# apachepinot/pinot

Measured on NVIDIA H100. Metric: scanned rows/sec for filter+groupby(3 dims,4 aggs) @1/2/4/8 H100; %HBM BW, higher is better.
Workload: dtype f64

## Files before the change

pinot_b200/csrc/pb_device.cuh:

```cuda
#pragma once
#include <cuda_runtime.h>
#include <stdint.h>

#define PB_NTHREADS 256
#define PB_NWARPS 8
#define PB_CHUNK_DOCS 1024
#define PB_NSTAGE 2
#define PB_MAX_LEAVES 16
#define PB_MAX_NODES 32
#define PB_MAX_GROUP_BY 16
#define PB_MAX_AGGS 16
#define PB_MAX_SCAN_SLOTS 8
#define PB_MAX_AGG_FILTERS 8
#define PB_MAX_AF_LEAVES 16
#define PB_MAX_AF_NODES 48
#define PB_SPARSE_MAX 128
#define PB_OUT_CAP 256
#define PB_CAND_CAP 512
#define PB_SET_SMEM_BYTES 8192

enum { L_TRUE = 0, L_FALSE = 1, L_DICT_RANGE = 2, L_DICT_SET = 3, L_RAW_RANGE_I = 4, L_RAW_RANGE_F = 5,
       L_RAW_SET = 6, L_BITMAP = 7 };
enum { N_LEAF = 0, N_AND = 1, N_OR = 2, N_NOT = 3 };
enum { T_KEYLESS = 0, T_DENSE = 1, T_HASH = 2 };
// ... 677 lines not shown
  __device__ __forceinline__ uint32_t fcnt(int k, uint32_t slot) const { return base + 4u * ((uint32_t)(1 + k) * S + slot); }
  __device__ __forceinline__ uint32_t acc(int k, uint32_t slot) const { return base + ((((1u + n_fc) * S * 4u) + 7u) & ~7u) + 8u * ((uint32_t)k * S + slot); }
};
__host__ __device__ __forceinline__ size_t pb_smem_table_bytes(uint32_t S, int n_fc, int n_acc) {
  return ((((size_t)(1 + n_fc) * S * 4 + 7) & ~(size_t)7) + (size_t)n_acc * S * 8 + 15) & ~(size_t)15;
}

__device__ __forceinline__ void pb_accumulate_smem(const DevQuery& Q, const DevSegQuery& sq, const DevTable& t, const SmemTable& st, uint32_t doc, uint32_t fpass) {
  const int nA = Q.n_aggs;
  uint64_t slot, slot_hi;
  double vals[PB_MAX_AGGS];
  pb_gather_doc(Q, sq, doc, slot, slot_hi, vals);
  const uint32_t sl = (uint32_t)slot;
  pb_sh_add_u32(st.cnt(sl), 1u);
  for (int a = 0; a < nA; a++) {
    const int op = Q.agg_op[a];
    const int fo = Q.agg_filter_of[a];
    if (fo >= 0) {
      if (!((fpass >> fo) & 1u)) continue;
      if (st.fc_of[a] >= 0) pb_sh_add_u32(st.fcnt(st.fc_of[a], sl), 1u);
    }
    if (op == 0) continue;
    const double v = vals[a];
    if (op == 5) {
      if (t.dset[a]) { pb_dset_insert(t, a, slot, (unsigned long long)__double_as_longlong(v)); continue; }
      uint32_t id = (uint32_t)__double_as_longlong(v);
      pb_red_or_b32(&t.dc_bits[a][slot * t.dc_words[a] + (id >> 5)], 1u << (id & 31));
      continue;
    }
    const uint32_t cell = st.acc(st.acc_of[a], sl);
    if (op == 1 || op == 4) {
      unsigned long long old = pb_sh_ld_u64(cell), assumed;
      do {
        assumed = old;
        old = pb_sh_cas_u64(cell, assumed, (unsigned long long)__double_as_longlong(__longlong_as_double((long long)assumed) + v));
      } while (old != assumed);
    } else if (v == v) {
      const long long e = op == 2 ? pb_enc_f64(v) : ~pb_enc_f64(v);
      long long old = (long long)pb_sh_ld_u64(cell);
      while (e < old) {
        const long long seen = (long long)pb_sh_cas_u64(cell, (unsigned long long)old, (unsigned long long)e);
        if (seen == old) break;
        old = seen;
      }
    }
  }
}

struct DevRowKey { uint32_t off, bits; uint64_t mult; const int32_t* remap; };
struct DevRowAgg { uint32_t off, width, type, exact_int; };
struct DevRowSeg {
  const uint32_t* rows;
  uint64_t doc_base;
  int32_t table, pad;
  DevRowKey keys[PB_MAX_GROUP_BY];
  DevRowAgg aggs[PB_MAX_AGGS];
};

template <int RW>
__device__ __forceinline__ void pb_load_row(const uint32_t* __restrict__ rows, unsigned long long doc, uint32_t (&w)[RW]) {
  const uint32_t* __restrict__ row = rows + doc * (unsigned long long)RW;
  if (RW == 2) { const uint2 v = __ldg(reinterpret_cast<const uint2*>(row)); w[0] = v.x; w[1 % RW] = v.y; }
  else {
#pragma unroll
    for (int q4 = 0; q4 < RW / 4; q4++) {
      const uint4 v = __ldg(reinterpret_cast<const uint4*>(row) + q4);
      w[(4 * q4) % RW] = v.x; w[(4 * q4 + 1) % RW] = v.y; w[(4 * q4 + 2) % RW] = v.z; w[(4 * q4 + 3) % RW] = v.w;
    }
  }
#pragma unroll
  for (int k = 0; k < RW; k++) w[k] = pb_bswap32(w[k]);
}

template <int RW>
__device__ __forceinline__ uint32_t pb_row_field(const uint32_t (&w)[RW], uint32_t off, uint32_t bits) {
  const uint32_t wi = off >> 5, sh = off & 31u;
  uint32_t hi = w[0], lo = RW > 1 ? w[1 % RW] : 0u;
#pragma unroll
  for (int k = 1; k < RW; k++) if (wi == (uint32_t)k) { hi = w[k]; lo = k + 1 < RW ? w[(k + 1) % RW] : 0u; }
  return __funnelshift_l(lo, hi, sh) >> (32u - bits);
}

template <int RW>
__device__ __forceinline__ uint64_t pb_row_slot(const uint32_t (&w)[RW], const DevRowSeg& sg, int nG) {
  uint64_t slot = 0;
  for (int j = 0; j < nG; j++) {
    const DevRowKey& k = sg.keys[j];
    uint32_t id = pb_row_field<RW>(w, k.off, k.bits);
    if (k.remap) id = (uint32_t)__ldg(k.remap + id);
    slot += (uint64_t)id * k.mult;
  }
  return slot;
}

template <int RW>
__device__ __forceinline__ double pb_row_value(const uint32_t (&w)[RW], const DevRowAgg& g) {
  const uint32_t w0 = pb_row_field<RW>(w, g.off, 32u);
  if (g.width == 4) return g.type == 2 ? (double)__uint_as_float(w0) : (double)(int32_t)w0;
  const unsigned long long u = ((unsigned long long)w0 << 32) | pb_row_field<RW>(w, g.off + 32u, 32u);
  return g.type == 3 ? __longlong_as_double((long long)u) : (double)(long long)u;
}
template <int RW>
__device__ __forceinline__ long long pb_row_ivalue(const uint32_t (&w)[RW], const DevRowAgg& g) {
  const uint32_t w0 = pb_row_field<RW>(w, g.off, 32u);
  if (g.width == 4) return (long long)(int32_t)w0;
  return (long long)(((unsigned long long)w0 << 32) | pb_row_field<RW>(w, g.off + 32u, 32u));
}

template <int RW>
__device__ __forceinline__ void pb_row_aggregate_global(const DevQuery& Q, const DevRowSeg& sg, const uint32_t (&w)[RW], uint64_t slot, uint32_t doc) {
  const DevTable& t = Q.tables[sg.table];
  pb_red_add_u64(&t.rowcnt[slot], 1ull);
  if (t.first_doc) asm volatile("red.global.min.u32 [%0], %1;" ::"l"(t.first_doc + slot), "r"(doc));
  for (int a = 0; a < Q.n_aggs; a++) {
    const int op = Q.agg_op[a];
    if (op == 0) continue;
    const double v = pb_row_value<RW>(w, sg.aggs[a]);
    if (op == 1 || op == 4) pb_red_add_f64(&t.sum[a][slot], v);
    else if (v == v) pb_red_min_s64(&t.mm[a][slot], op == 2 ? pb_enc_f64(v) : ~pb_enc_f64(v));
  }
}

struct __align__(16) FilterSmemHeader {
  uint64_t full[PB_NWARPS][PB_NSTAGE];
  uint32_t slot_stride[PB_MAX_SCAN_SLOTS];
  uint32_t slot_last_rel[PB_MAX_SCAN_SLOTS];
  uint32_t n_scan_full_bytes;
  int32_t flat_and;
  int32_t n_flat;
  int32_t flat_leaf[PB_MAX_LEAVES];
  int32_t n_dense;
  int32_t pad_g;
  alignas(16) uint8_t seg[PB_SEG_FILTER_BYTES];
};

template <int U, int MIN_CTAS, int SW = 0, int SPK = 0, int RW = 0>
__global__ void __launch_bounds__(PB_NTHREADS, MIN_CTAS) pb_filter_kernel(const __grid_constant__ DevQuery Q) {
  extern __shared__ __align__(128) uint8_t smem_raw[];
  FilterSmemHeader* H = reinterpret_cast<FilterSmemHeader*>(smem_raw);
  const int tid = threadIdx.x, lane = tid & 31, warp = tid >> 5;
  uint8_t* dyn = smem_raw + ((sizeof(FilterSmemHeader) + 127) & ~(size_t)127);
  DevRowSeg* rseg = reinterpret_cast<DevRowSeg*>(dyn);
  if constexpr (RW > 0) dyn += (sizeof(DevRowSeg) + 127) & ~(size_t)127;
  uint8_t* set_cache = dyn;
  dyn += (Q.set_cache_bytes + 127) & ~127;
  uint16_t* cand = reinterpret_cast<uint16_t*>(dyn);
  dyn += Q.cand_bytes;
  const uint32_t OUT_CAP = (uint32_t)Q.out_cap, CAND_CAP = (uint32_t)Q.cand_cap;
  uint32_t* ob = reinterpret_cast<uint32_t*>(dyn) + (size_t)warp * OUT_CAP;
  dyn += (size_t)PB_NWARPS * OUT_CAP * sizeof(uint32_t);
  uint32_t out_n = 0;
  auto flush_out = [&]() {
    if (out_n == 0) return;
    __syncwarp();
    unsigned long long base = 0;
    if (lane == 0) base = atomicAdd(Q.match_count, (unsigned long long)out_n);
    base = __shfl_sync(0xffffffffu, base, 0);
    for (uint32_t i = (uint32_t)lane; i < out_n; i += 32) Q.match_list[base + i] = ob[i];
    __syncwarp();
    out_n = 0;
  };
  uint8_t* my_stages = dyn + (size_t)warp * PB_NSTAGE * Q.stage_bytes;
  const bool staged = Q.stage_bytes > 0;
  constexpr uint32_t UNIT_DOCS = U * PB_CHUNK_DOCS;

  if (lane == 0)
    for (int s = 0; s < PB_NSTAGE; s++) pb_mbar_init(&H->full[warp][s], 1);
  asm volatile("fence.mbarrier_init.release.cluster;" ::: "memory");
  __syncthreads();

  const uint64_t per = (Q.n_units + gridDim.x - 1) / gridDim.x;
  const uint64_t cta_lo = Q.unit_lo + (uint64_t)blockIdx.x * per;
  const uint64_t cta_hi = cta_lo + per < Q.unit_lo + Q.n_units ? cta_lo + per : Q.unit_lo + Q.n_units;
  if (cta_lo >= cta_hi) return;
  int seg_first = 0;
  while (seg_first + 1 < Q.n_segs && cta_lo >= Q.segs[seg_first + 1].unit_begin) seg_first++;

  uint32_t consumed = 0;
  const DevSegQuery& sq = *reinterpret_cast<const DevSegQuery*>(H->seg);
  const uint64_t l2_stream = pb_policy_evict_first();

  auto eval_leaf = [&](const DevLeaf& lf, const uint8_t* stage, uint64_t unit_doc0, int nu, const uint32_t* restrict_to, bool sparse, uint32_t* m) {
    switch (lf.kind) {
      case L_TRUE: for (int u = 0; u < nu; u++) m[u] = 0xffffffffu; return;
      case L_FALSE: for (int u = 0; u < nu; u++) m[u] = 0u; return;
      case L_DICT_RANGE: {
        const uint32_t* p = reinterpret_cast<const uint32_t*>(stage + Q.slot_off[lf.slot]);
        PredRange pr; pr.lo = lf.lo; pr.span = lf.span;
        if (sparse) { for (int u = 0; u < nu; u++) m[u] = pb_eval_dict_sparse<PredRange>(p + u * 32 * lf.bits, lf.bits, pr, lane, restrict_to[u]); return; }
        pb_eval_dict<PredRange>(p, lf.bits, pr, lane, Q.generic, nu, m);
        return;
      }
      case L_DICT_SET: {
        const uint32_t* p = reinterpret_cast<const uint32_t*>(stage + Q.slot_off[lf.slot]);
        if (lf.set_smem_off >= 0) {
          PredLut8 pl; pl.lut = set_cache + lf.set_smem_off;
          if (sparse) { for (int u = 0; u < nu; u++) m[u] = pb_eval_dict_sparse<PredLut8>(p + u * 32 * lf.bits, lf.bits, pl, lane, restrict_to[u]); return; }
          pb_eval_dict<PredLut8>(p, lf.bits, pl, lane, Q.generic, nu, m);
          return;
        }
        PredBits pb; pb.bits = lf.set_bits; pb.excl = (uint32_t)lf.exclusive;
        if (sparse) { for (int u = 0; u < nu; u++) m[u] = pb_eval_dict_sparse<PredBits>(p + u * 32 * lf.bits, lf.bits, pb, lane, restrict_to[u]); return; }
        pb_eval_dict<PredBits>(p, lf.bits, pb, lane, Q.generic, nu, m);
        return;
      }
      case L_RAW_RANGE_I:
      case L_RAW_RANGE_F:
      case L_RAW_SET: {
        const uint32_t* p = reinterpret_cast<const uint32_t*>(stage + Q.slot_off[lf.slot]);
        for (int u = 0; u < nu; u++) m[u] = pb_eval_raw(p + u * (PB_CHUNK_DOCS / 4) * lf.raw_width, lf, lane);
        return;
      }
      default: {
        for (int u = 0; u < nu; u++) {
          uint32_t w = __ldg(lf.bitmap + (unit_doc0 >> 5) + u * 32 + lane);
          m[u] = lf.exclusive ? ~w : w;
        }
        return;
      }
    }
  };

  for (int sgi = seg_first; sgi < Q.n_segs; sgi++) {
    if (Q.segs[sgi].unit_begin >= cta_hi) break;
    __syncthreads();
    {
      const uint32_t* src = reinterpret_cast<const uint32_t*>(&Q.segs[sgi]);
      uint32_t* dst = reinterpret_cast<uint32_t*>(H->seg);
      for (int i = tid; i < (int)(PB_SEG_FILTER_BYTES / 4); i += PB_NTHREADS) dst[i] = src[i];
      if constexpr (RW > 0) {
        const uint32_t* rsrc = reinterpret_cast<const uint32_t*>(Q.row_segs + sgi);
        uint32_t* rdst = reinterpret_cast<uint32_t*>(rseg);
        for (int i = tid; i < (int)(sizeof(DevRowSeg) / 4); i += PB_NTHREADS) rdst[i] = rsrc[i];
      }
      __syncthreads();
      if (tid < sq.n_scan) {
        const uint32_t stride = (uint32_t)(UNIT_DOCS / 8) * (uint32_t)sq.scan[tid].bits_per_doc;
        H->slot_stride[tid] = stride;
        const uint64_t total = sq.scan[tid].bytes_total;
        H->slot_last_rel[tid] = total >= (uint64_t)stride + 16 ? (uint32_t)((total - stride - 16) / stride) + 1 : 0u;
      }
      if (tid == 96) {
        uint32_t t = 0;
        for (int c = 0; c < sq.n_scan; c++) t += (uint32_t)(UNIT_DOCS / 8) * (uint32_t)sq.scan[c].bits_per_doc + 16;
        H->n_scan_full_bytes = t;
      }
      if (tid == 64) {
        int nl = 0; bool flat = true;
        for (int n = 0; n < sq.n_nodes; n++) {
          if (sq.node_kind[n] == N_LEAF) { if (nl < PB_MAX_LEAVES) H->flat_leaf[nl] = sq.node_arg[n]; nl++; }
          else if (!(sq.node_kind[n] == N_AND && n == sq.n_nodes - 1 && sq.node_arg[n] == nl)) flat = false;
        }
        int nd = 0;
        if (flat && nl <= PB_MAX_LEAVES) {
          auto key = [&](int l) { return sq.leaves[l].est_permille + (sq.leaves[l].gather ? 4096 : 0); };
          for (int a = 1; a < nl; a++) {
            int x = H->flat_leaf[a]; int b = a - 1;
            while (b >= 0 && key(H->flat_leaf[b]) > key(x)) { H->flat_leaf[b + 1] = H->flat_leaf[b]; b--; }
            H->flat_leaf[b + 1] = x;
          }
          for (int a = 0; a < nl; a++) if (!sq.leaves[H->flat_leaf[a]].gather) nd++;
        }
        H->flat_and = flat ? 1 : 0;
        H->n_flat = nl;
        H->n_dense = nd;
      }
      for (int l = 0; l < PB_MAX_LEAVES; l++) {
        const DevLeaf& lf = sq.leaves[l];
        if (lf.kind == L_DICT_SET && lf.set_smem_off >= 0) {
          for (int i = tid; i < lf.set_card; i += PB_NTHREADS)
            set_cache[lf.set_smem_off + i] = (uint8_t)(((__ldg(lf.set_bits + (i >> 5)) >> (i & 31)) & 1u) ^ (uint32_t)lf.exclusive);
        }
      }
      __syncthreads();
    }
    const uint64_t seg_lo = sq.unit_begin > cta_lo ? sq.unit_begin : cta_lo;
    const uint64_t seg_end = sq.unit_begin + sq.n_units;
    const uint64_t seg_hi = seg_end < cta_hi ? seg_end : cta_hi;
    const uint64_t first = seg_lo + warp;
    const uint32_t n_mine = first < seg_hi ? (uint32_t)((seg_hi - first + PB_NWARPS - 1) / PB_NWARPS) : 0u;
    const uint32_t rel0 = (uint32_t)(first - sq.unit_begin);
    const int n_scan = sq.n_scan;
    unsigned long long matched = 0;
    uint32_t min_last_rel = 0xffffffffu;
    for (int c = 0; c < n_scan; c++) min_last_rel = min(min_last_rel, H->slot_last_rel[c]);

    auto issue = [&](uint32_t k, uint32_t seq) {
      const uint32_t rel = rel0 + k * PB_NWARPS;
      const int st = (int)(seq % PB_NSTAGE);
      uint8_t* dst = my_stages + (size_t)st * Q.stage_bytes;
      uint64_t* bar = &H->full[warp][st];
      if (__builtin_expect(rel < min_last_rel, 1)) {
        pb_mbar_expect_tx(bar, H->n_scan_full_bytes);
        for (int c = 0; c < n_scan; c++) {
          const uint32_t stride = H->slot_stride[c];
          pb_tma_load_1d_hint(dst + Q.slot_off[c], sq.scan[c].base + (uint64_t)rel * stride, stride + 16, bar, l2_stream);
        }
        return;
      }
      uint32_t total = 0;
      uint32_t nbytes[PB_MAX_SCAN_SLOTS];
      for (int c = 0; c < n_scan; c++) {
        const uint64_t off = (uint64_t)rel * H->slot_stride[c];
        const uint64_t want = (uint64_t)H->slot_stride[c] + 16;
        const uint64_t avail = sq.scan[c].bytes_total - off;
        nbytes[c] = (uint32_t)((want < avail ? want : avail) & ~(uint64_t)15);
        total += nbytes[c];
      }
      pb_mbar_expect_tx(bar, total);
      for (int c = 0; c < n_scan; c++)
        pb_tma_load_1d(dst + Q.slot_off[c], sq.scan[c].base + (uint64_t)rel * H->slot_stride[c], nbytes[c], bar);
    };

    if (staged && Q.use_tma && lane == 0)
      for (uint32_t k = 0; k < PB_NSTAGE - 1 && k < n_mine; k++) issue(k, consumed + k);

    for (uint32_t k = 0; k < n_mine; k++) {
      const uint64_t unit_doc0 = (uint64_t)(rel0 + k * PB_NWARPS) * UNIT_DOCS;
      const int st = (int)(consumed % PB_NSTAGE);
      uint8_t* stage = my_stages + (size_t)st * Q.stage_bytes;
      if (staged) {
        if (__builtin_expect(Q.use_tma != 0, 1)) {
          if (lane == 0 && k + PB_NSTAGE - 1 < n_mine) issue(k + PB_NSTAGE - 1, consumed + PB_NSTAGE - 1);
          pb_mbar_wait(&H->full[warp][st], (consumed / PB_NSTAGE) & 1u);
        } else {
          for (int c = 0; c < n_scan; c++) {
            const uint64_t off = (uint64_t)(rel0 + k * PB_NWARPS) * H->slot_stride[c];
            const uint64_t want = (uint64_t)H->slot_stride[c] + 16;
            const uint64_t avail = sq.scan[c].bytes_total - off;
            const uint64_t n = (want < avail ? want : avail) & ~(uint64_t)15;
            const uint4* s4 = reinterpret_cast<const uint4*>(sq.scan[c].base + off);
            uint4* d4 = reinterpret_cast<uint4*>(stage + Q.slot_off[c]);
            for (uint32_t i = lane; i < (uint32_t)(n / 16); i += 32) d4[i] = __ldg(s4 + i);
          }
          __syncwarp();
        }
      }
      consumed++;

      uint32_t mask[U], tmp[U];
      int nu = 0;
      const uint32_t nd_rel = (uint32_t)sq.num_docs - (uint32_t)unit_doc0;
      nu = nd_rel >= (uint32_t)U * PB_CHUNK_DOCS ? U : (int)((nd_rel + PB_CHUNK_DOCS - 1) / PB_CHUNK_DOCS);
#pragma unroll
      for (int u = 0; u < U; u++) {
        const uint32_t d = (uint32_t)u * PB_CHUNK_DOCS + 32u * (uint32_t)lane;
        mask[u] = nd_rel >= d + 32u ? 0xffffffffu : (nd_rel <= d ? 0u : ((1u << (nd_rel - d)) - 1u));
      }
      const int n_cand_leaves = H->flat_and ? H->n_flat - H->n_dense : 0;
      if constexpr (SW > 0) {
        const DevLeaf& lf = sq.leaves[H->flat_leaf[0]];
        const uint32_t* p = reinterpret_cast<const uint32_t*>(stage + Q.slot_off[lf.slot]);
        if constexpr (SPK == 0) {
          PredRange pr; pr.lo = lf.lo; pr.span = lf.span;
#pragma unroll
          for (int u = 0; u < U; u++) if (u < nu) mask[u] &= pb_eval_dict_w<SW, PredRange>(p + u * 32 * SW, pr, lane);
        } else {
          PredLut8 pl; pl.lut = set_cache + lf.set_smem_off;
#pragma unroll
          for (int u = 0; u < U; u++) if (u < nu) mask[u] &= pb_eval_dict_w<SW, PredLut8>(p + u * 32 * SW, pl, lane);
        }
      } else if (__builtin_expect(H->flat_and != 0, 1)) {
        const int nl = H->n_dense;
        for (int i = 0; i < nl; i++) {
          uint32_t pc = 0;
#pragma unroll
          for (int u = 0; u < U; u++) pc += (uint32_t)__popc(mask[u]);
          const bool sparse = i > 0 && !Q.generic && __reduce_add_sync(0xffffffffu, pc) <= (uint32_t)Q.sparse_max * U;
          eval_leaf(sq.leaves[H->flat_leaf[i]], stage, unit_doc0, nu, mask, sparse, tmp);
          uint32_t any = 0;
#pragma unroll
          for (int u = 0; u < U; u++) { if (u < nu) mask[u] &= tmp[u]; any |= mask[u]; }
          if (sparse && !__any_sync(0xffffffffu, any != 0)) break;
        }
      } else {
        uint32_t stack[PB_MAX_LEAVES][U];
        const uint32_t all[2] = {0xffffffffu, 0xffffffffu};
        int sp = 0;
        for (int n = 0; n < sq.n_nodes; n++) {
          const int kind = sq.node_kind[n], arg = sq.node_arg[n];
          if (kind == N_LEAF) { eval_leaf(sq.leaves[arg], stage, unit_doc0, nu, all, false, stack[sp]); sp++; }
          else if (kind == N_NOT) { for (int u = 0; u < nu; u++) stack[sp - 1][u] = ~stack[sp - 1][u]; }
          else {
            for (int u = 0; u < nu; u++) {
              uint32_t r = stack[sp - arg][u];
              for (int i = 1; i < arg; i++) r = (kind == N_AND) ? (r & stack[sp - arg + i][u]) : (r | stack[sp - arg + i][u]);
              stack[sp - arg][u] = r;
            }
            sp -= arg - 1;
          }
        }
        if (sp > 0) for (int u = 0; u < nu; u++) mask[u] &= stack[0][u];
      }
      __syncwarp();

      uint32_t cnt = 0;
#pragma unroll
      for (int u = 0; u < U; u++) cnt += (uint32_t)__popc(mask[u]);
      const uint32_t mx = __reduce_max_sync(0xffffffffu, cnt);
      if (mx == 0) continue;
      uint32_t excl = 0, total = 0;
      const uint32_t lt = (1u << lane) - 1u;
      if (mx <= 4) {
        for (uint32_t kk = 1; kk <= mx; kk++) {
          const uint32_t b = __ballot_sync(0xffffffffu, cnt >= kk);
          excl += __popc(b & lt);
          total += __popc(b);
        }
      } else {
        uint32_t incl = cnt;
#pragma unroll
        for (int o = 1; o < 32; o <<= 1) { uint32_t t = __shfl_up_sync(0xffffffffu, incl, o); if (lane >= o) incl += t; }
        total = __shfl_sync(0xffffffffu, incl, 31);
        excl = incl - cnt;
      }
      const uint32_t gunit0 = (uint32_t)(sq.doc_base + unit_doc0);
      if (RW == 0 && n_cand_leaves == 0) {
        if (__builtin_expect(total > OUT_CAP, 0)) {
          unsigned long long base = 0;
          if (lane == 0) base = atomicAdd(Q.match_count, (unsigned long long)total);
          base = __shfl_sync(0xffffffffu, base, 0);
          uint32_t* out = Q.match_list + base + excl;
#pragma unroll
          for (int u = 0; u < U; u++) {
            const uint32_t gdoc0 = gunit0 + (uint32_t)u * PB_CHUNK_DOCS + 32u * (uint32_t)lane;
            uint32_t mm = mask[u];
            while (mm) {
              const int bit = __ffs(mm) - 1;
              mm &= mm - 1;
              *out++ = gdoc0 + (uint32_t)bit;
            }
          }
        } else {
          if (out_n + total > OUT_CAP) flush_out();
          uint32_t* out = ob + out_n + excl;
#pragma unroll
          for (int u = 0; u < U; u++) {
            const uint32_t gdoc0 = gunit0 + (uint32_t)u * PB_CHUNK_DOCS + 32u * (uint32_t)lane;
            uint32_t mm = mask[u];
            while (mm) {
              const int bit = __ffs(mm) - 1;
              mm &= mm - 1;
              *out++ = gdoc0 + (uint32_t)bit;
            }
          }
          out_n += total;
        }
        matched += total;
      } else {
        uint16_t* cl = cand + (size_t)warp * CAND_CAP;
        for (uint32_t pass0 = 0; pass0 < total; pass0 += CAND_CAP) {
          if (pass0) __syncwarp();
          {
            uint32_t pos = excl - pass0;
#pragma unroll
            for (int u = 0; u < U; u++) {
              const uint32_t off0 = (uint32_t)u * PB_CHUNK_DOCS + 32u * (uint32_t)lane;
              uint32_t mm = mask[u];
              while (mm) {
                const int bit = __ffs(mm) - 1;
                mm &= mm - 1;
                if (pos < CAND_CAP) cl[pos] = (uint16_t)(off0 + (uint32_t)bit);
                pos++;
              }
            }
          }
          __syncwarp();
          const uint32_t n_pass = total - pass0 < CAND_CAP ? total - pass0 : CAND_CAP;
          for (uint32_t b0 = 0; b0 < n_pass; b0 += 32) {
            const uint32_t idx = b0 + (uint32_t)lane;
            bool alive = idx < n_pass;
            const uint32_t off = alive ? (uint32_t)cl[idx] : 0u;
            const uint32_t doc = (uint32_t)unit_doc0 + off;
            if constexpr (RW > 0) {
              uint32_t w[RW];
              if (alive) pb_load_row<RW>(rseg->rows, doc, w);
              for (int i = 0; i < n_cand_leaves; i++) {
                const DevLeaf& lf = sq.leaves[H->flat_leaf[H->n_dense + i]];
                if (alive) alive = pb_dict_leaf_test(lf, set_cache, pb_row_field<RW>(w, (uint32_t)lf.g_bit_off, (uint32_t)lf.bits));
              }
              if (alive) pb_row_aggregate_global<RW>(Q, *rseg, w, pb_row_slot<RW>(w, *rseg, Q.n_group_by), doc);
              matched += (uint32_t)__popc(__ballot_sync(0xffffffffu, alive));
            } else {
              for (int i = 0; i < n_cand_leaves; i++) {
                if (alive) alive = pb_leaf_test_doc(sq.leaves[H->flat_leaf[H->n_dense + i]], set_cache, doc);
                if (!__any_sync(0xffffffffu, alive)) break;
              }
              const uint32_t bal = __ballot_sync(0xffffffffu, alive);
              if (bal) {
                const uint32_t n = (uint32_t)__popc(bal);
                if (out_n + n > OUT_CAP) flush_out();
                if (alive) ob[out_n + __popc(bal & lt)] = gunit0 + off;
                out_n += n;
                matched += n;
              }
            }
          }
        }
        __syncwarp();
      }
    }
    flush_out();
    if (lane == 0 && matched) pb_red_add_u64(Q.tables[sq.table].docs_matched, matched);
  }
}

#define PB_AGG_MAX_SEGS_SMEM 1024

template <int MIN_CTAS>
__global__ void __launch_bounds__(PB_NTHREADS, MIN_CTAS) pb_agg_kernel(const __grid_constant__ DevQuery Q) {
  extern __shared__ __align__(128) uint8_t smem_raw[];
  const int tid = threadIdx.x, lane = tid & 31, warp = tid >> 5;
  __shared__ unsigned long long s_doc_base[PB_AGG_MAX_SEGS_SMEM + 1];
  __shared__ unsigned long long s_red_u64[PB_NWARPS];
  __shared__ double s_red_f64[PB_NWARPS];
  __shared__ long long s_red_i64[PB_NWARPS];
  __shared__ int s_table0;
  const int n_segs = Q.n_segs;
  const int n_smem = n_segs < PB_AGG_MAX_SEGS_SMEM ? n_segs : PB_AGG_MAX_SEGS_SMEM;
  for (int i = tid; i < n_smem; i += PB_NTHREADS) s_doc_base[i] = Q.segs[i].doc_base;
  KeylessAcc ka;
  ka.sum = nullptr; ka.mm = nullptr; ka.cnt = nullptr;
  const long long ENC_POS_INF = 0x7ff0000000000000LL;
  const long long ENC_NEG_INF = (long long)0xfff0000000000000ULL ^ 0x7fffffffffffffffLL;
  const bool keyless = Q.table_mode == T_KEYLESS;
  if (keyless) {
    ka.sum = reinterpret_cast<double*>(smem_raw);
    ka.mm = reinterpret_cast<long long*>(smem_raw + sizeof(double) * Q.n_aggs * PB_NTHREADS);
    if (Q.n_agg_filters > 0) ka.cnt = reinterpret_cast<unsigned long long*>(smem_raw + 2 * sizeof(double) * Q.n_aggs * PB_NTHREADS);
    for (int a = 0; a < Q.n_aggs; a++) {
      ka.sum[a * PB_NTHREADS + tid] = 0.0;
      ka.mm[a * PB_NTHREADS + tid] = Q.agg_op[a] == 2 ? ENC_POS_INF : ENC_NEG_INF;
      if (ka.cnt) ka.cnt[a * PB_NTHREADS + tid] = 0ull;
    }
  }
  __syncthreads();

  if (Q.phase == 2 && *Q.any_limit == 0) return;
  const unsigned long long n = Q.match_all ? Q.n_docs_total : *Q.match_count;
  unsigned long long keyless_rows = 0;
  int my_table = -1;

  auto keyless_flush_thread = [&]() {
    if (my_table < 0) return;
    const DevTable& t = Q.tables[my_table];
    if (keyless_rows) pb_red_add_u64(&t.rowcnt[0], keyless_rows);
    keyless_rows = 0;
    for (int a = 0; a < Q.n_aggs; a++) {
      const int op = Q.agg_op[a];
      if (op == 1 || op == 4) { pb_red_add_f64(&t.sum[a][0], ka.sum[a * PB_NTHREADS + tid]); ka.sum[a * PB_NTHREADS + tid] = 0.0; }
      else if (op == 2) { pb_red_min_s64(&t.mm[a][0], ka.mm[a * PB_NTHREADS + tid]); ka.mm[a * PB_NTHREADS + tid] = ENC_POS_INF; }
      else if (op == 3) { pb_red_min_s64(&t.mm[a][0], ~ka.mm[a * PB_NTHREADS + tid]); ka.mm[a * PB_NTHREADS + tid] = ENC_NEG_INF; }
      if (ka.cnt && t.fcnt[a]) { if (ka.cnt[a * PB_NTHREADS + tid]) pb_red_add_u64(&t.fcnt[a][0], ka.cnt[a * PB_NTHREADS + tid]); ka.cnt[a * PB_NTHREADS + tid] = 0ull; }
    }
  };
  const int nF = Q.n_agg_filters;
  int stat_seg = -1;
  unsigned int stat_cnt[1 + PB_MAX_AGG_FILTERS];
#pragma unroll
  for (int f = 0; f <= PB_MAX_AGG_FILTERS; f++) stat_cnt[f] = 0;
  auto stat_flush = [&]() {
    if (stat_seg < 0) return;
    unsigned long long* dst = Q.segs[stat_seg].af_docs;
#pragma unroll
    for (int f = 0; f <= PB_MAX_AGG_FILTERS; f++) if (f <= nF && stat_cnt[f]) { pb_red_add_u64(dst + f, (unsigned long long)stat_cnt[f]); stat_cnt[f] = 0; }
  };

  for (unsigned long long i = (unsigned long long)blockIdx.x * PB_NTHREADS + tid; i < n; i += (unsigned long long)gridDim.x * PB_NTHREADS) {
    const unsigned long long gdoc = Q.match_all ? i : (unsigned long long)__ldg(Q.match_list + i);
    int lo = 0, hi = n_segs - 1;
    while (lo < hi) {
      const int mid = (lo + hi + 1) >> 1;
      const unsigned long long b = mid < PB_AGG_MAX_SEGS_SMEM ? s_doc_base[mid] : Q.segs[mid].doc_base;
      if (b <= gdoc) lo = mid; else hi = mid - 1;
    }
    const DevSegQuery& sg = Q.segs[lo];
    const uint32_t doc = (uint32_t)(gdoc - (lo < PB_AGG_MAX_SEGS_SMEM ? s_doc_base[lo] : sg.doc_base));
    const int table = sg.table;
    if (keyless && table != my_table) { keyless_flush_thread(); my_table = table; }
    uint32_t fpass = 0;
    if (nF > 0) {
      fpass = pb_agg_filter_bits(sg, doc);
      if (Q.phase != 2) {
        if (lo != stat_seg) { stat_flush(); stat_seg = lo; }
        stat_cnt[0]++;
// ... 921 lines not shown
```

pinot_b200/csrc/pb_engine.cu:

```cuda
#include "../../include/pinot_b200.h"
#include "pb_device.cuh"
#include "pb_filter_spec.h"

#include <dlfcn.h>
#include <nccl.h>

#include <algorithm>
#include <chrono>
#include <cmath>
#include <cstdarg>
#include <cstdio>
#include <cstring>
#include <map>
#include <memory>
#include <mutex>
#include <string>
#include <unordered_set>
#include <vector>

static thread_local char g_err[1024];
static int fail(int code, const char* fmt, ...) {
  va_list ap;
  va_start(ap, fmt);
  vsnprintf(g_err, sizeof g_err, fmt, ap);
// ... 2372 lines not shown
      w.dq.match_count = P.hq->match_count + waves.size();
      w.n_units = w.dq.n_units; w.n_docs = w.dq.n_docs_total;
      waves.push_back(w);
    }
  } else {
    for (int si = 0; si < n_segs; si++) if (P.seg_wait[si]) CU(cudaStreamWaitEvent(P.st, P.seg_wait[si], 0));
    pb_result_s::WaveLaunch w;
    w.dq = *P.hq; w.seg_lo = 0; w.seg_hi = n_segs; w.n_units = P.n_chunks; w.n_docs = P.n_docs_total;
    waves.push_back(w);
  }
  return PB_OK;
}

static int upload_descriptors(Plan& P) {
  pb_result_s* r = P.r;
  CU(cudaMemcpyAsync(P.ar.dev, P.ar.host.data(), P.ar.used, cudaMemcpyHostToDevice, P.st));
  const uint64_t zn = (P.zero_bytes + 15) / 16, fn = (P.ff_bytes + 15) / 16, mn = (8 * P.mm_elems + 15) / 16, an = (P.aux_bytes + 15) / 16;
  const uint64_t mx = std::max(std::max(zn, an), std::max(fn, mn));
  int grid = (int)std::min<uint64_t>((mx + 255) / 256, (uint64_t)P.ctx->num_sms * 8);
  if (grid < 1) grid = 1;
  long long* d_mm = P.mm_elems ? reinterpret_cast<long long*>(P.d_zero + P.zero_bytes) : nullptr;
  r->init = {(uint4*)P.d_zero, zn, (uint4*)P.d_ff, fn, (uint4*)d_mm, mn, (uint4*)P.d_aux, an, reinterpret_cast<const uint4*>(P.d_head),
             (uint64_t)PB_COUNTERS_PER_TABLE * P.n_tables / 2, grid};
  return PB_OK;
}

static size_t filter_smem(const Plan& P, int out_cap, int cand_cap) {
  return ((sizeof(FilterSmemHeader) + 127) & ~(size_t)127) + (((size_t)P.set_cache_max + 127) & ~(size_t)127) + (P.any_cand_leaf ? (size_t)2 * cand_cap * PB_NWARPS : 0) +
         (size_t)PB_NWARPS * out_cap * 4 + P.stage_bytes * PB_NSTAGE * PB_NWARPS;
}

static void plan_filter_spec(Plan& P, size_t& smem, uint64_t& max_ctas) {
  static const bool spec_on = []() { const char* e = getenv("PB_FILTER_SPEC"); return !e || atoi(e) != 0; }();
  pb_result_s::Replay& rp = P.r->rp;
  if (!(spec_on && !P.match_all && P.n_chunks > 0 && rp.U == 2 && rp.u2_three && !P.hq->generic && P.hq->use_tma)) return;
  int w = -1, pk = -1;
  for (int si = 0; si < P.n_segs; si++) {
    const DevSegQuery& ds = P.hsegs[si];
    int nl = 0, dense = -1, n_dense = 0;
    for (int n = 0; n < ds.n_nodes; n++) {
      if (ds.node_kind[n] == N_LEAF) {
        const DevLeaf& lf = ds.leaves[ds.node_arg[n]];
        if (!lf.gather) { dense = ds.node_arg[n]; n_dense++; }
        nl++;
      } else if (!(ds.node_kind[n] == N_AND && n == ds.n_nodes - 1 && ds.node_arg[n] == nl)) return;
    }
    if (n_dense != 1) return;
    const DevLeaf& lf = ds.leaves[dense];
    const int k = lf.kind == L_DICT_RANGE ? 0 : (lf.kind == L_DICT_SET && lf.set_smem_off >= 0) ? 1 : -1;
    if (k < 0 || (w >= 0 && (w != lf.bits || pk != k))) return;
    w = lf.bits; pk = k;
  }
  if (w <= 0 || !pb_filter_spec_available(w, pk)) return;
  size_t smem_spec = smem;
  int oc = PB_OUT_CAP, cc = PB_CAND_CAP;
  if (4 * (filter_smem(P, PB_OUT_CAP / 2, PB_CAND_CAP / 2) + 1024) <= 227 * 1024 && 4 * (smem + 1024) > 227 * 1024) { oc /= 2; cc /= 2; smem_spec = filter_smem(P, oc, cc); }
  int occ = 0;
  if (pb_filter_spec_prepare(w, pk, 0, smem_spec, &occ) == cudaSuccess && occ >= 1) {
    rp.spec_w = w; rp.spec_pk = pk; max_ctas = (uint64_t)P.ctx->num_sms * (uint64_t)occ; smem = smem_spec;
    P.hq->out_cap = oc; P.hq->cand_cap = cc; P.hq->cand_bytes = P.any_cand_leaf ? (int32_t)(2 * cc * PB_NWARPS) : 0;
    for (auto& wv : rp.waves) { wv.dq.out_cap = oc; wv.dq.cand_cap = cc; wv.dq.cand_bytes = P.hq->cand_bytes; }
  } else cudaGetLastError();
}

static bool plan_fused_agg(Plan& P, size_t& smem, uint64_t& max_ctas) {
  static const bool fused_on = []() { const char* e = getenv("PB_FUSED_AGG"); return !e || atoi(e) != 0; }();
  pb_result_s* r = P.r;
  pb_result_s::Replay& rp = r->rp;
  if (!(fused_on && rp.spec_w > 0 && P.any_cand_leaf && P.d_row_segs && !r->track_first && P.nF == 0 && r->table_mode == T_DENSE &&
        rp.waves.size() == 1)) return false;
  double expected = 0;
  for (int si = 0; si < P.n_segs; si++) {
    const DevSegQuery& ds = P.hsegs[si];
    for (int n = 0; n < ds.n_nodes; n++) {
      if (ds.node_kind[n] != N_LEAF) continue;
      const DevLeaf& lf = ds.leaves[ds.node_arg[n]];
      const bool row_field = (lf.kind == L_DICT_RANGE || lf.kind == L_DICT_SET) && (const void*)lf.gfwd == (const void*)P.h_row_segs[si].rows &&
                             lf.g_stride_bits == 32 * P.rows_rw;
      if (lf.gather && !row_field) return false;
    }
    expected += estimate_selectivity(P.g->segs[si], P.sqs[si]) * (double)P.g->segs[si]->num_docs;
  }
  if (P.st_replicas > 0 && expected >= (double)P.hq->st_min_docs) return false;
  const size_t smem_fused = filter_smem(P, 0, P.hq->cand_cap) + ((sizeof(DevRowSeg) + 127) & ~(size_t)127);
  int occ = 0;
  if (pb_filter_spec_prepare(rp.spec_w, rp.spec_pk, P.rows_rw, smem_fused, &occ) != cudaSuccess || occ < 1) { cudaGetLastError(); return false; }
  smem = smem_fused; max_ctas = (uint64_t)P.ctx->num_sms * (uint64_t)occ;
  P.hq->out_cap = 0; P.hq->row_segs = P.d_row_segs;
  for (auto& wv : rp.waves) { wv.dq.out_cap = 0; wv.dq.row_segs = P.d_row_segs; }
  return true;
}

static int plan_launches(Plan& P) {
  Context* ctx = P.ctx;
  pb_result_s* r = P.r;
  pb_result_s::Replay& rp = r->rp;
  {
    std::lock_guard<std::mutex> lk(ctx->mu);
    if (!ctx->smem_attr_set) {
      CU(cudaFuncSetAttribute(pb_filter_kernel<1, 3>, cudaFuncAttributeMaxDynamicSharedMemorySize, 227 * 1024));
      CU(cudaFuncSetAttribute(pb_filter_kernel<2, 2>, cudaFuncAttributeMaxDynamicSharedMemorySize, 227 * 1024));
      CU(cudaFuncSetAttribute(pb_filter_kernel<2, 3>, cudaFuncAttributeMaxDynamicSharedMemorySize, 227 * 1024));
      CU(cudaFuncSetAttribute(pb_agg_kernel<6>, cudaFuncAttributeMaxDynamicSharedMemorySize, 96 * 1024));
      CU(cudaFuncSetAttribute(pb_agg_smem_kernel, cudaFuncAttributeMaxDynamicSharedMemorySize, 227 * 1024 - 16 * 1024));
      for (const void* k : {(const void*)pb_agg_rows_kernel<2>, (const void*)pb_agg_rows_kernel<4>, (const void*)pb_agg_rows_kernel<8>}) {
        cudaFuncAttributes fa;
        CU(cudaFuncGetAttributes(&fa, k));
        CU(cudaFuncSetAttribute(k, cudaFuncAttributeMaxDynamicSharedMemorySize, 227 * 1024 - (int)fa.sharedSizeBytes));
      }
      ctx->smem_attr_set = true;
    }
  }
  rp.U = P.U;
  size_t smem = 0;
  uint64_t max_ctas = 0;
  if (!P.match_all && P.n_chunks > 0) {
    smem = filter_smem(P, PB_OUT_CAP, PB_CAND_CAP);
    if (smem > 227 * 1024) return fail(PB_ERR_UNSUPPORTED, "filter kernel needs %zu bytes of shared memory", smem);
    int occ = 1;
    rp.u2_three = P.U == 2 && 3 * (smem + 1024) <= 227 * 1024;
    if (P.U == 1) CU(cudaOccupancyMaxActiveBlocksPerMultiprocessor(&occ, pb_filter_kernel<1, 3>, PB_NTHREADS, smem));
    else if (rp.u2_three) CU(cudaOccupancyMaxActiveBlocksPerMultiprocessor(&occ, pb_filter_kernel<2, 3>, PB_NTHREADS, smem));
    else CU(cudaOccupancyMaxActiveBlocksPerMultiprocessor(&occ, pb_filter_kernel<2, 2>, PB_NTHREADS, smem));
    if (occ < 1) return fail(PB_ERR_CUDA, "filter kernel does not fit an SM (smem %zu)", smem);
    max_ctas = (uint64_t)ctx->num_sms * (uint64_t)occ;
  }
  plan_filter_spec(P, smem, max_ctas);
  const bool fused = plan_fused_agg(P, smem, max_ctas);
  rp.smem_filter = smem;
  const bool use_smem_table = P.st_replicas > 0;
  const size_t smem2 = r->table_mode == T_KEYLESS ? (P.nF > 0 ? 3 : 2) * sizeof(double) * (size_t)P.nA * PB_NTHREADS : 0;
  uint64_t max2 = 0;
  if (P.n_docs_total > 0 && !use_smem_table) {
    int occ2 = 1;
    CU(cudaOccupancyMaxActiveBlocksPerMultiprocessor(&occ2, pb_agg_kernel<6>, PB_NTHREADS, smem2));
    if (occ2 < 1) return fail(PB_ERR_CUDA, "aggregation kernel does not fit an SM");
    max2 = (uint64_t)ctx->num_sms * (uint64_t)occ2;
  }
  rp.expand_items = P.d_expand_items; rp.n_expand = (int)P.expand_items.size();
  rp.agg = P.n_docs_total == 0 ? AGG_NONE : fused ? AGG_FUSED : P.d_row_segs ? AGG_ROWS : use_smem_table ? AGG_SMEM : AGG_GENERAL;
  const bool smem_threads = rp.agg == AGG_SMEM || rp.agg == AGG_ROWS;
  rp.smem_agg = (use_smem_table && smem_threads) ? (size_t)P.st_replicas * P.st_rep_bytes : rp.agg == AGG_ROWS ? 0 : smem2;
  rp.row_segs = P.d_row_segs; rp.rows_rw = P.rows_rw;
  rp.lane_w = P.d_lane_w; rp.n_lanes = 1 + P.nF; rp.n_segs = P.n_segs;
  for (auto& wl : rp.waves) {
    wl.grid_filter = (!P.match_all && wl.n_units > 0) ? (int)std::min<uint64_t>(std::max<uint64_t>((wl.n_units + PB_NWARPS - 1) / PB_NWARPS, 1), max_ctas) : 0;
    if (wl.n_docs == 0 || rp.agg == AGG_NONE || rp.agg == AGG_FUSED) wl.grid_agg = 0;
    else if (smem_threads) wl.grid_agg = (int)std::min<uint64_t>(std::max<uint64_t>((wl.n_docs + PB_AGG_SMEM_THREADS - 1) / PB_AGG_SMEM_THREADS, 1), (uint64_t)ctx->num_sms);
    else wl.grid_agg = (int)std::min<uint64_t>(std::max<uint64_t>((wl.n_docs + PB_NTHREADS - 1) / PB_NTHREADS, 1), max2);
  }
  bool small = true;
  for (auto& tm : r->tables) if (tm.capacity + 1 > (1ull << 20)) small = false;
  rp.cacheable = P.n_pending == 0 && !P.in_place && rp.waves.size() == 1 && small && !(P.q->flags & PB_Q_DEFER_FINALIZE) && r->in_place_columns == 0;
  int32_t* pi = r->plan_info;
  const int st_replicas = fused ? 0 : P.st_replicas;
  pi[0] = (int32_t)(fused ? AGG_ROWS : rp.agg); pi[1] = (rp.agg == AGG_ROWS || fused) ? rp.rows_rw : 0;
  pi[2] = st_replicas; pi[3] = st_replicas > 0 ? (int32_t)std::min<uint64_t>(P.hq->st_min_docs, INT32_MAX) : 0;
  pi[4] = r->table_mode; pi[5] = r->key_words;
  pi[6] = (P.match_all || P.n_chunks == 0) ? 0 : rp.spec_w > 0 ? 3 : rp.U;
  pi[7] = rp.spec_w; pi[8] = rp.spec_w > 0 ? rp.spec_pk : 0;
  pi[9] = P.any_cand_leaf ? 1 : 0;
  pi[10] = 0;
  if (P.h_row_segs && st_replicas > 0) for (int a = 0; a < P.nA; a++) if (P.h_row_segs[0].aggs[a].exact_int) pi[10] |= 1 << a;
  pi[11] = fused ? 1 : 0;
  return PB_OK;
}

static int exec_single(pb_segment_group_handle g, const pb_segment_query* sqs, const pb_query_desc* q, pb_result_handle* out) {
  int rc = validate_query(g, sqs, q);
  if (rc) return rc;

  std::string sig;
// ... 783 lines not shown
```

Measured before the change: 442.1 billion.

## Compact fused filter matches into per-warp ring and prefetch rows via cp.async

In the fused filter+aggregate path, matching doc ids are compacted into a per-warp ring buffer in shared memory. Full 32-doc rounds then have their row records fetched asynchronously with cp.async, so the gather for the next round overlaps the aggregation of the previous one. Field extraction offsets are precomputed per segment into shared memory, and rows are decoded from shared memory instead of registers. This replaces per-candidate-chunk loads with dense, full-warp rounds to cut idle lanes and exposed gather latency. The cost is extra shared memory per warp and more warp syncs.

```diff
diff --git a/pinot_b200/csrc/pb_device.cuh b/pinot_b200/csrc/pb_device.cuh
--- a/pinot_b200/csrc/pb_device.cuh
+++ b/pinot_b200/csrc/pb_device.cuh
@@ -783,24 +783,50 @@
 }
 
 template <int RW>
-__device__ __forceinline__ uint64_t pb_row_slot(const uint32_t (&w)[RW], const DevRowSeg& sg, int nG) {
+__device__ __forceinline__ uint32_t pb_row_field_at(uint32_t off, uint32_t bits) {
+  uint32_t wi = off >> 5;
+  if (wi >= (uint32_t)RW) wi = RW - 1;
+  if (bits > 32u) bits = 32u;
+  const uint32_t sh = off & 31u, lo = sh + bits > 32u && wi + 1 < (uint32_t)RW ? (wi + 1) * 4u : 0xffu;
+  return wi * 4u | lo << 8 | sh << 16 | (32u - bits) << 24;
+}
+__device__ __forceinline__ uint32_t pb_row_field_smem(const uint8_t* row, uint32_t f) {
+  const uint32_t hi = pb_bswap32(*reinterpret_cast<const uint32_t*>(row + (f & 0xffu)));
+  const uint32_t lb = (f >> 8) & 0xffu;
+  const uint32_t lo = lb != 0xffu ? pb_bswap32(*reinterpret_cast<const uint32_t*>(row + lb)) : 0u;
+  return __funnelshift_l(lo, hi, (f >> 16) & 0xffu) >> (f >> 24);
+}
+
+template <int RW>
+struct RegRow {
+  const uint32_t (&w)[RW];
+  __device__ __forceinline__ uint32_t key(const DevRowKey& k, int) const { return pb_row_field<RW>(w, k.off, k.bits); }
+  __device__ __forceinline__ uint32_t word(const DevRowAgg& g, int, int h) const { return pb_row_field<RW>(w, g.off + 32u * (uint32_t)h, 32u); }
+};
+
+template <class R>
+__device__ __forceinline__ uint64_t pb_row_slot(const R& r, const DevRowSeg& sg, int nG) {
   uint64_t slot = 0;
   for (int j = 0; j < nG; j++) {
     const DevRowKey& k = sg.keys[j];
-    uint32_t id = pb_row_field<RW>(w, k.off, k.bits);
+    uint32_t id = r.key(k, j);
     if (k.remap) id = (uint32_t)__ldg(k.remap + id);
     slot += (uint64_t)id * k.mult;
   }
   return slot;
 }
-
 template <int RW>
-__device__ __forceinline__ double pb_row_value(const uint32_t (&w)[RW], const DevRowAgg& g) {
-  const uint32_t w0 = pb_row_field<RW>(w, g.off, 32u);
+__device__ __forceinline__ uint64_t pb_row_slot(const uint32_t (&w)[RW], const DevRowSeg& sg, int nG) { return pb_row_slot(RegRow<RW>{w}, sg, nG); }
+
+template <class R>
+__device__ __forceinline__ double pb_row_value(const R& r, const DevRowAgg& g, int a) {
+  const uint32_t w0 = r.word(g, a, 0);
   if (g.width == 4) return g.type == 2 ? (double)__uint_as_float(w0) : (double)(int32_t)w0;
-  const unsigned long long u = ((unsigned long long)w0 << 32) | pb_row_field<RW>(w, g.off + 32u, 32u);
+  const unsigned long long u = ((unsigned long long)w0 << 32) | r.word(g, a, 1);
   return g.type == 3 ? __longlong_as_double((long long)u) : (double)(long long)u;
 }
+template <int RW>
+__device__ __forceinline__ double pb_row_value(const uint32_t (&w)[RW], const DevRowAgg& g) { return pb_row_value(RegRow<RW>{w}, g, 0); }
 template <int RW>
 __device__ __forceinline__ long long pb_row_ivalue(const uint32_t (&w)[RW], const DevRowAgg& g) {
   const uint32_t w0 = pb_row_field<RW>(w, g.off, 32u);
@@ -808,19 +834,53 @@
   return (long long)(((unsigned long long)w0 << 32) | pb_row_field<RW>(w, g.off + 32u, 32u));
 }
 
-template <int RW>
-__device__ __forceinline__ void pb_row_aggregate_global(const DevQuery& Q, const DevRowSeg& sg, const uint32_t (&w)[RW], uint64_t slot, uint32_t doc) {
+template <class R>
+__device__ __forceinline__ void pb_row_aggregate_global(const DevQuery& Q, const DevRowSeg& sg, const R& r, uint64_t slot, uint32_t doc) {
   const DevTable& t = Q.tables[sg.table];
   pb_red_add_u64(&t.rowcnt[slot], 1ull);
   if (t.first_doc) asm volatile("red.global.min.u32 [%0], %1;" ::"l"(t.first_doc + slot), "r"(doc));
   for (int a = 0; a < Q.n_aggs; a++) {
     const int op = Q.agg_op[a];
     if (op == 0) continue;
-    const double v = pb_row_value<RW>(w, sg.aggs[a]);
+    const double v = pb_row_value(r, sg.aggs[a], a);
     if (op == 1 || op == 4) pb_red_add_f64(&t.sum[a][slot], v);
     else if (v == v) pb_red_min_s64(&t.mm[a][slot], op == 2 ? pb_enc_f64(v) : ~pb_enc_f64(v));
   }
 }
+template <int RW>
+__device__ __forceinline__ void pb_row_aggregate_global(const DevQuery& Q, const DevRowSeg& sg, const uint32_t (&w)[RW], uint64_t slot, uint32_t doc) {
+  pb_row_aggregate_global(Q, sg, RegRow<RW>{w}, slot, doc);
+}
+
+struct FusedSegSmem {
+  DevRowSeg seg;
+  uint32_t cand[PB_MAX_LEAVES];
+  uint32_t key[PB_MAX_GROUP_BY];
+  uint32_t val[PB_MAX_AGGS][2];
+};
+struct SmemRow {
+  const uint8_t* row;
+  const FusedSegSmem& fs;
+  __device__ __forceinline__ uint32_t key(const DevRowKey&, int j) const { return pb_row_field_smem(row, fs.key[j]); }
+  __device__ __forceinline__ uint32_t word(const DevRowAgg&, int a, int h) const { return pb_row_field_smem(row, fs.val[a][h]); }
+};
+#define PB_FQ_CAP 128
+#define PB_FQ_WIN (PB_FQ_CAP - 32)
+__host__ __device__ constexpr size_t pb_fused_warp_bytes(int rw) { return (size_t)32 * 4 * rw + 32 * 4 + PB_FQ_CAP * 4; }
+
+template <int RW>
+__device__ __forceinline__ void pb_cp_async_row(uint32_t* dst, const uint32_t* rows, uint32_t doc) {
+  const uint32_t d = (uint32_t)__cvta_generic_to_shared(dst);
+  const size_t s = __cvta_generic_to_global(rows + (size_t)doc * RW);
+  if constexpr (RW == 2) {
+    asm volatile("cp.async.ca.shared.global [%0], [%1], 8;" ::"r"(d), "l"(s) : "memory");
+  } else {
+#pragma unroll
+    for (int q = 0; q < RW / 4; q++) asm volatile("cp.async.cg.shared.global [%0], [%1], 16;" ::"r"(d + 16u * q), "l"(s + 16u * q) : "memory");
+  }
+}
+__device__ __forceinline__ void pb_cp_async_commit() { asm volatile("cp.async.commit_group;" ::: "memory"); }
+__device__ __forceinline__ void pb_cp_async_wait_all() { asm volatile("cp.async.wait_group 0;" ::: "memory"); }
 
 struct __align__(16) FilterSmemHeader {
   uint64_t full[PB_NWARPS][PB_NSTAGE];
@@ -841,11 +901,15 @@
   FilterSmemHeader* H = reinterpret_cast<FilterSmemHeader*>(smem_raw);
   const int tid = threadIdx.x, lane = tid & 31, warp = tid >> 5;
   uint8_t* dyn = smem_raw + ((sizeof(FilterSmemHeader) + 127) & ~(size_t)127);
-  DevRowSeg* rseg = reinterpret_cast<DevRowSeg*>(dyn);
-  if constexpr (RW > 0) dyn += (sizeof(DevRowSeg) + 127) & ~(size_t)127;
+  FusedSegSmem* fseg = reinterpret_cast<FusedSegSmem*>(dyn);
+  DevRowSeg* rseg = &fseg->seg;
+  if constexpr (RW > 0) dyn += (sizeof(FusedSegSmem) + 127) & ~(size_t)127;
   uint8_t* set_cache = dyn;
   dyn += (Q.set_cache_bytes + 127) & ~127;
   uint16_t* cand = reinterpret_cast<uint16_t*>(dyn);
+  uint32_t* f_rows = reinterpret_cast<uint32_t*>(dyn + (size_t)warp * pb_fused_warp_bytes(RW));
+  uint32_t* f_docs = f_rows + 32 * RW;
+  uint32_t* f_ring = f_docs + 32;
   dyn += Q.cand_bytes;
   const uint32_t OUT_CAP = (uint32_t)Q.out_cap, CAND_CAP = (uint32_t)Q.cand_cap;
   uint32_t* ob = reinterpret_cast<uint32_t*>(dyn) + (size_t)warp * OUT_CAP;
@@ -935,6 +999,12 @@
         for (int i = tid; i < (int)(sizeof(DevRowSeg) / 4); i += PB_NTHREADS) rdst[i] = rsrc[i];
       }
       __syncthreads();
+      if constexpr (RW > 0) {
+        if (tid < PB_MAX_LEAVES) fseg->cand[tid] = pb_row_field_at<RW>((uint32_t)sq.leaves[tid].g_bit_off, (uint32_t)sq.leaves[tid].bits);
+        if (tid >= 128 && tid < 128 + PB_MAX_GROUP_BY) fseg->key[tid - 128] = pb_row_field_at<RW>(rseg->keys[tid - 128].off, rseg->keys[tid - 128].bits);
+        if (tid >= 160 && tid < 160 + 2 * PB_MAX_AGGS)
+          fseg->val[(tid - 160) >> 1][tid & 1] = pb_row_field_at<RW>(rseg->aggs[(tid - 160) >> 1].off + 32u * (uint32_t)(tid & 1), 32u);
+      }
       if (tid < sq.n_scan) {
         const uint32_t stride = (uint32_t)(UNIT_DOCS / 8) * (uint32_t)sq.scan[tid].bits_per_doc;
         H->slot_stride[tid] = stride;
@@ -986,6 +1056,27 @@
     uint32_t min_last_rel = 0xffffffffu;
     for (int c = 0; c < n_scan; c++) min_last_rel = min(min_last_rel, H->slot_last_rel[c]);
 
+    uint32_t q_head = 0, q_n = 0;
+    bool in_flight = false;
+    auto stage_round = [&](uint32_t doc, bool live) {
+      f_docs[lane] = doc;
+      if (live) pb_cp_async_row<RW>(f_rows + lane * RW, rseg->rows, doc);
+      pb_cp_async_commit();
+    };
+    auto consume_round = [&](bool live) {
+      pb_cp_async_wait_all();
+      const uint32_t doc = f_docs[lane];
+      const SmemRow r{reinterpret_cast<const uint8_t*>(f_rows + lane * RW), *fseg};
+      bool alive = live;
+      const int n_cand = H->flat_and ? H->n_flat - H->n_dense : 0;
+      for (int i = 0; i < n_cand; i++) {
+        const int l = H->flat_leaf[H->n_dense + i];
+        if (alive) alive = pb_dict_leaf_test(sq.leaves[l], set_cache, pb_row_field_smem(r.row, fseg->cand[l]));
+      }
+      if (alive) pb_row_aggregate_global(Q, *rseg, r, pb_row_slot(r, *rseg, Q.n_group_by), doc);
+      matched += (uint32_t)__popc(__ballot_sync(0xffffffffu, alive));
+    };
+
     auto issue = [&](uint32_t k, uint32_t seq) {
       const uint32_t rel = rel0 + k * PB_NWARPS;
       const int st = (int)(seq % PB_NSTAGE);
@@ -999,18 +1090,17 @@
         }
         return;
       }
-      uint32_t total = 0;
-      uint32_t nbytes[PB_MAX_SCAN_SLOTS];
-      for (int c = 0; c < n_scan; c++) {
+      auto nbytes = [&](int c) -> uint32_t {
         const uint64_t off = (uint64_t)rel * H->slot_stride[c];
         const uint64_t want = (uint64_t)H->slot_stride[c] + 16;
         const uint64_t avail = sq.scan[c].bytes_total - off;
-        nbytes[c] = (uint32_t)((want < avail ? want : avail) & ~(uint64_t)15);
-        total += nbytes[c];
-      }
+        return (uint32_t)((want < avail ? want : avail) & ~(uint64_t)15);
+      };
+      uint32_t total = 0;
+      for (int c = 0; c < n_scan; c++) total += nbytes(c);
       pb_mbar_expect_tx(bar, total);
       for (int c = 0; c < n_scan; c++)
-        pb_tma_load_1d(dst + Q.slot_off[c], sq.scan[c].base + (uint64_t)rel * H->slot_stride[c], nbytes[c], bar);
+        pb_tma_load_1d(dst + Q.slot_off[c], sq.scan[c].base + (uint64_t)rel * H->slot_stride[c], nbytes(c), bar);
     };
 
     if (staged && Q.use_tma && lane == 0)
@@ -1116,7 +1206,32 @@
         excl = incl - cnt;
       }
       const uint32_t gunit0 = (uint32_t)(sq.doc_base + unit_doc0);
-      if (RW == 0 && n_cand_leaves == 0) {
+      if constexpr (RW > 0) {
+        __syncwarp();
+        for (uint32_t pass0 = 0; pass0 < total; pass0 += PB_FQ_WIN) {
+          if (pass0) __syncwarp();
+          uint32_t pos = excl - pass0;
+          const uint32_t at = q_head + q_n;
+#pragma unroll
+          for (int u = 0; u < U; u++) {
+            const uint32_t doc0 = (uint32_t)unit_doc0 + (uint32_t)u * PB_CHUNK_DOCS + 32u * (uint32_t)lane;
+            uint32_t mm = mask[u];
+            while (mm) {
+              const int bit = __ffs(mm) - 1;
+              mm &= mm - 1;
+              if (pos < PB_FQ_WIN) f_ring[(at + pos) & (PB_FQ_CAP - 1)] = doc0 + (uint32_t)bit;
+              pos++;
+            }
+          }
+          __syncwarp();
+          q_n += total - pass0 < PB_FQ_WIN ? total - pass0 : PB_FQ_WIN;
+          while (q_n >= 32) {
+            if (in_flight) consume_round(true);
+            stage_round(f_ring[(q_head + lane) & (PB_FQ_CAP - 1)], true);
+            in_flight = true; q_head += 32; q_n -= 32;
+          }
+        }
+      } else if (n_cand_leaves == 0) {
         if (__builtin_expect(total > OUT_CAP, 0)) {
           unsigned long long base = 0;
           if (lane == 0) base = atomicAdd(Q.match_count, (unsigned long long)total);
@@ -1173,28 +1288,17 @@
             bool alive = idx < n_pass;
             const uint32_t off = alive ? (uint32_t)cl[idx] : 0u;
             const uint32_t doc = (uint32_t)unit_doc0 + off;
-            if constexpr (RW > 0) {
-              uint32_t w[RW];
-              if (alive) pb_load_row<RW>(rseg->rows, doc, w);
-              for (int i = 0; i < n_cand_leaves; i++) {
-                const DevLeaf& lf = sq.leaves[H->flat_leaf[H->n_dense + i]];
-                if (alive) alive = pb_dict_leaf_test(lf, set_cache, pb_row_field<RW>(w, (uint32_t)lf.g_bit_off, (uint32_t)lf.bits));
-              }
-              if (alive) pb_row_aggregate_global<RW>(Q, *rseg, w, pb_row_slot<RW>(w, *rseg, Q.n_group_by), doc);
-              matched += (uint32_t)__popc(__ballot_sync(0xffffffffu, alive));
-            } else {
-              for (int i = 0; i < n_cand_leaves; i++) {
-                if (alive) alive = pb_leaf_test_doc(sq.leaves[H->flat_leaf[H->n_dense + i]], set_cache, doc);
-                if (!__any_sync(0xffffffffu, alive)) break;
-              }
-              const uint32_t bal = __ballot_sync(0xffffffffu, alive);
-              if (bal) {
-                const uint32_t n = (uint32_t)__popc(bal);
-                if (out_n + n > OUT_CAP) flush_out();
-                if (alive) ob[out_n + __popc(bal & lt)] = gunit0 + off;
-                out_n += n;
-                matched += n;
-              }
+            for (int i = 0; i < n_cand_leaves; i++) {
+              if (alive) alive = pb_leaf_test_doc(sq.leaves[H->flat_leaf[H->n_dense + i]], set_cache, doc);
+              if (!__any_sync(0xffffffffu, alive)) break;
+            }
+            const uint32_t bal = __ballot_sync(0xffffffffu, alive);
+            if (bal) {
+              const uint32_t n = (uint32_t)__popc(bal);
+              if (out_n + n > OUT_CAP) flush_out();
+              if (alive) ob[out_n + __popc(bal & lt)] = gunit0 + off;
+              out_n += n;
+              matched += n;
             }
           }
         }
@@ -1202,6 +1306,14 @@
       }
     }
     flush_out();
+    if constexpr (RW > 0) {
+      if (in_flight) consume_round(true);
+      if (q_n) {
+        __syncwarp();
+        stage_round(f_ring[(q_head + lane) & (PB_FQ_CAP - 1)], (uint32_t)lane < q_n);
+        consume_round((uint32_t)lane < q_n);
+      }
+    }
     if (lane == 0 && matched) pb_red_add_u64(Q.tables[sq.table].docs_matched, matched);
   }
 }
diff --git a/pinot_b200/csrc/pb_engine.cu b/pinot_b200/csrc/pb_engine.cu
--- a/pinot_b200/csrc/pb_engine.cu
+++ b/pinot_b200/csrc/pb_engine.cu
@@ -2478,12 +2478,13 @@
     expected += estimate_selectivity(P.g->segs[si], P.sqs[si]) * (double)P.g->segs[si]->num_docs;
   }
   if (P.st_replicas > 0 && expected >= (double)P.hq->st_min_docs) return false;
-  const size_t smem_fused = filter_smem(P, 0, P.hq->cand_cap) + ((sizeof(DevRowSeg) + 127) & ~(size_t)127);
+  const int32_t fused_bytes = (int32_t)(PB_NWARPS * pb_fused_warp_bytes(P.rows_rw));
+  const size_t smem_fused = filter_smem(P, 0, 0) + ((sizeof(FusedSegSmem) + 127) & ~(size_t)127) + (size_t)fused_bytes;
   int occ = 0;
   if (pb_filter_spec_prepare(rp.spec_w, rp.spec_pk, P.rows_rw, smem_fused, &occ) != cudaSuccess || occ < 1) { cudaGetLastError(); return false; }
   smem = smem_fused; max_ctas = (uint64_t)P.ctx->num_sms * (uint64_t)occ;
-  P.hq->out_cap = 0; P.hq->row_segs = P.d_row_segs;
-  for (auto& wv : rp.waves) { wv.dq.out_cap = 0; wv.dq.row_segs = P.d_row_segs; }
+  P.hq->out_cap = 0; P.hq->row_segs = P.d_row_segs; P.hq->cand_bytes = fused_bytes;
+  for (auto& wv : rp.waves) { wv.dq.out_cap = 0; wv.dq.row_segs = P.d_row_segs; wv.dq.cand_bytes = fused_bytes; }
   return true;
 }
 
```

Measured after the change: 495.4 billion (median of 6 runs). 12.1% higher.
